# AIBluefisher/DReg-NeRF

Hardware: AMD Instinct MI355X
Metric: nerf_pairs_per_sec_regtr_fwd_bwd_128 (higher is better)
Workload: dtype bf16; 1 GPU; RegTR fwd+bwd+AdamW, shell-R synthetic pairs, 128^3 grids, 4 pairs (8 grids) per GPU per step, random-init weights; global_batch_pairs=4, resolution=128, fpn_head=active-set (identical results; rows around occupied voxels), parallelism=dp1

## Files before the change

### dreg_nerf_amd/csrc/pointset_exec.hip

```cpp
#include <hip/hip_runtime.h>
#include <cstdint>
#include <cstring>
#include <algorithm>
#include <vector>
#include "../../include/dreg_nerf.h"
#ifndef DREG_ELAUNCH
#define DREG_ELAUNCH (-2)
#endif

namespace {

constexpr int E = 256, E3 = 768, FF = 1024, NL = 6, NH = 8;
enum { N1W, N1B, SIW, SIB, SOW, SOB, N2W, N2B, CIW, CIB, COW, COB, N3W, N3B, L1W, L1B, L2W, L2B, PL_COUNT };
enum { FNW = NL * PL_COUNT, FNB, QW, QB, KW, KB, CW, CB, PS_NPARAM };
enum { LIN_SI, LIN_SO, LIN_CI, LIN_CO, LIN_1, LIN_2, LIN_PER_LAYER };
constexpr int NLIN = NL * LIN_PER_LAYER + 2;

struct Lin { int cout, cin, w, b; };
struct ReduceRec { const float* part; float* dw; int nsplit, Cout, Kpad, ntaps, Cin, Cin_real, accumulate, block0; };
static_assert(sizeof(ReduceRec) == 48, "matches WgradReduceDesc of conv.hip");
struct ColsumRec { const void* g; float* out; float* partial; int M, C, rpc, nch, pblock0, fblock0, accumulate, pad; };
static_assert(sizeof(ColsumRec) == 56, "matches ColsumDesc of fpn_ops.hip");
struct LnRec { const float* part; float* dg; float* db; int nblk, accumulate; };
static_assert(sizeof(LnRec) == 32, "matches LnFinalDesc of pointset.hip");

inline size_t al(size_t v) { return (v + 255) / 256 * 256; }

struct LayerBuf {
    size_t xa, xb, st1, st2, st3, h1, h2, h3, qkv1, qkv2, o1, o2, lse1, lse2, f;
    size_t gF, gB, gQ2, gC, gQ1;
    size_t wg[LIN_PER_LAYER], cs[LIN_PER_LAYER], lnp[3];
};
struct Layout {
    int R = -1;
    size_t allx, stf, dec_in, q, k, corr_lse;
    LayerBuf L[NL];
    size_t dallx, dallx_bf, dq, dk, ddec, ddec2, dH, dO, dvec, gx[2], lnpf[2], wgq, wgk, csq, csk, ov_ws, ks_ws, cs_ws, tables;
    size_t ks_bytes = 0, total = 0;
    size_t wg_bytes[NLIN];
};

struct Ps {
    float* val[PS_NPARAM];
    float* grad[PS_NPARAM];
    Lin lin[NLIN];
    Layout lay;
    int fuse = 1;
    int group_wgrad = 1;
    std::vector<hipEvent_t> ev;
    hipEvent_t ev_done = nullptr;
    static constexpr int RING = 8;
    static constexpr size_t TABLE_BYTES = 16384;
    char* pinned = nullptr;
    hipEvent_t ring_ev[RING] = {};
    unsigned ring_next = 0;
    struct Timed { hipEvent_t e0, e1; int kind, rows, cin, cout, flags; };
    bool timing = false;
    std::vector<Timed> timed;
    size_t timed_used = 0;
};

struct PsScope {
    Ps::Timed* t = nullptr; hipStream_t st;
    PsScope(Ps* p, void* stream, int kind, int rows, int cin, int cout, int flags) : st((hipStream_t)stream) {
        if (!p->timing) return;
        if (p->timed_used == p->timed.size()) {
            Ps::Timed n{};
            if (hipEventCreate(&n.e0) != hipSuccess || hipEventCreate(&n.e1) != hipSuccess) return;
            p->timed.push_back(n);
        }
        t = &p->timed[p->timed_used++];
        t->kind = kind; t->rows = rows; t->cin = cin; t->cout = cout; t->flags = flags;
        (void)hipEventRecord(t->e0, st);
    }
    ~PsScope() { if (t) (void)hipEventRecord(t->e1, st); }
};

inline int lin_index(int layer, int which) { return layer * LIN_PER_LAYER + which; }

void build_layout(Ps* p, int R)
{
    Layout& y = p->lay;
    if (y.R == R) return;
    y = Layout();
    y.R = R;
    size_t off = 0;
    auto take = [&](size_t bytes) { const size_t o = off; off += al(bytes); return o; };
    const size_t r = (size_t)R;
    y.allx = take(NL * r * E * 4);
    y.stf = take(NL * r * 2 * 4);
    y.dec_in = take(NL * r * E * 2);
    y.q = take(NL * r * E * 2);
    y.k = take(NL * r * E * 2);
    y.corr_lse = take(NL * r * 4);
    for (int i = 0; i < NLIN; ++i) {
        const Lin& l = p->lin[i];
        const int rows = i < NL * LIN_PER_LAYER ? R : NL * R;
        y.wg_bytes[i] = dreg_conv3d_wgrad_workspace_bytes(rows, 1, 1, 1, l.cin, l.cout, 1, 0);
        const size_t k1 = dreg_conv3d_igemm_workspace_bytes(rows, 1, 1, 1, l.cin, 1, 1, 1, l.cout, 1, 1, 0, 0, 0, 0);
        const size_t k2 = dreg_conv3d_igemm_workspace_bytes(rows, 1, 1, 1, l.cout, 1, 1, 1, l.cin, 1, 1, 0, 1, 0, 0);
// ... 39 lines not shown
int linear_fwd(Ps* p, const Layout& y, char* A, const void* x, const void* wpk, const float* bias, const void* residual, void* out,
               int rows, int cin, int cout, int relu, int out_f32, void* st)
{
    PsScope sc(p, st, 0, rows, cin, cout, (residual ? 1 : 0) | (out_f32 ? 2 : 0) | (y.ks_bytes ? 4 : 0));
    return dreg_conv3d_igemm_ws(x, wpk, out, bias, residual, rows, 1, 1, 1, cin, 1, 1, 1, cout, 1, 1, 0, 0, relu, residual ? 1 : 0, residual ? 1 : 0,
                                residual ? 1 : 0, residual ? 1 : 0, 0, out_f32, y.ks_bytes ? A + y.ks_ws : nullptr, y.ks_bytes, st);
}
int linear_dgrad(Ps* p, const Layout& y, char* A, const void* g, const void* wpk_t, void* gx, const void* mask, const void* add,
                 int rows, int cin, int cout, void* st)
{
    const void* addend = mask ? mask : add;
    PsScope sc(p, st, 1, rows, cin, cout, (addend ? 1 : 0) | (y.ks_bytes ? 4 : 0));
    return dreg_conv3d_igemm_ws(g, wpk_t, gx, nullptr, addend, rows, 1, 1, 1, cout, 1, 1, 1, cin, 1, 1, 0, 1, mask ? 2 : 0, addend ? 1 : 0, addend ? 1 : 0,
                                addend ? 1 : 0, addend ? 1 : 0, 0, 0, y.ks_bytes ? A + y.ks_ws : nullptr, y.ks_bytes, st);
}

}

extern "C" {

int dreg_ps_num_params(void) { return PS_NPARAM; }
int dreg_ps_num_linears(void) { return NLIN; }

void* dreg_ps_create(const int64_t* params)
{
    Ps* p = new Ps();
    for (int i = 0; i < PS_NPARAM; ++i) { p->val[i] = (float*)params[2 * i]; p->grad[i] = (float*)params[2 * i + 1]; }
    for (int l = 0; l < NL; ++l) {
        const int o = l * PL_COUNT;
        p->lin[lin_index(l, LIN_SI)] = {E3, E, o + SIW, o + SIB};
        p->lin[lin_index(l, LIN_SO)] = {E, E, o + SOW, o + SOB};
        p->lin[lin_index(l, LIN_CI)] = {E3, E, o + CIW, o + CIB};
        p->lin[lin_index(l, LIN_CO)] = {E, E, o + COW, o + COB};
        p->lin[lin_index(l, LIN_1)] = {FF, E, o + L1W, o + L1B};
        p->lin[lin_index(l, LIN_2)] = {E, FF, o + L2W, o + L2B};
    }
    p->lin[NLIN - 2] = {E, E, QW, QB};
    p->lin[NLIN - 1] = {E, E, KW, KB};
    if (hipHostMalloc((void**)&p->pinned, Ps::RING * Ps::TABLE_BYTES, hipHostMallocDefault) != hipSuccess) { delete p; return nullptr; }
    return p;
}
void dreg_ps_destroy(void* h)
{
    Ps* p = (Ps*)h;
    if (!p) return;
    for (auto& e : p->ev) if (e) (void)hipEventDestroy(e);
    if (p->ev_done) (void)hipEventDestroy(p->ev_done);
    for (auto& e : p->ring_ev) if (e) (void)hipEventDestroy(e);
    for (auto& t : p->timed) { (void)hipEventDestroy(t.e0); (void)hipEventDestroy(t.e1); }
    if (p->pinned) (void)hipHostFree(p->pinned);
    delete p;
}
void dreg_ps_set_fuse(void* h, int fuse) { ((Ps*)h)->fuse = fuse ? 1 : 0; }
void dreg_ps_set_group_wgrad(void* h, int on) { ((Ps*)h)->group_wgrad = on ? 1 : 0; }
void dreg_ps_set_timing(void* h, int enable) { ((Ps*)h)->timing = enable != 0; }
int dreg_ps_read_timings(void* h, int* info, float* ms, int cap)
{
    Ps* p = (Ps*)h;
    int n = 0;
    for (size_t i = 0; i < p->timed_used && n < cap; ++i) {
        const Ps::Timed& t = p->timed[i];
        float v = 0.f;
        if (hipEventElapsedTime(&v, t.e0, t.e1) != hipSuccess) continue;
        info[5 * n] = t.kind; info[5 * n + 1] = t.rows; info[5 * n + 2] = t.cin; info[5 * n + 3] = t.cout; info[5 * n + 4] = t.flags;
        ms[n++] = v;
    }
    p->timed_used = 0;
    return n;
}
size_t dreg_ps_arena_bytes(void* h, int R) { Ps* p = (Ps*)h; build_layout(p, R); return p->lay.total; }

int dreg_ps_forward(void* h, void* arena, size_t arena_bytes, const int64_t* packs, const float* feats, const float* xyz, const float* pe,
                    const int* probs_self, const int* probs_cross, int nprob, int max_len, int R,
                    float* cond, float* corr, float* ov, void* stream)
{
    Ps* p = (Ps*)h;
    if (R <= 0) return DREG_EINVAL;
    build_layout(p, R);
    const Layout& y = p->lay;
    if (arena_bytes < y.total) return DREG_EINVAL;
    char* A = (char*)arena;
    const float sc = 0.17677669529663687f;
    auto pk = [&](int li, int t) { return (const void*)packs[2 * li + t]; };
    const float* xin = feats;
    for (int l = 0; l < NL; ++l) {
        const LayerBuf& b = y.L[l];
        const int o = l * PL_COUNT;
        float* xout = (float*)(A + y.allx) + (size_t)l * R * E;
        CK(dreg_layernorm_fwd(xin, p->val[o + N1W], p->val[o + N1B], pe, A + b.h1, (float*)(A + b.st1), R, E, 1e-5f, 0, stream));
        CK(linear_fwd(p, y, A, A + b.h1, pk(lin_index(l, LIN_SI), 0), p->val[o + SIB], nullptr, A + b.qkv1, R, E, E3, 0, 0, stream));
        CK(dreg_mha_varlen_fwd(A + b.qkv1, A + b.qkv1 + E * 2, A + b.qkv1 + 2 * E * 2, A + b.o1, (float*)(A + b.lse1), probs_self, nprob, max_len, max_len,
                               R, NH, E3, E3, E3, E, sc, 0, stream));
        CK(linear_fwd(p, y, A, A + b.o1, pk(lin_index(l, LIN_SO), 0), p->val[o + SOB], xin, A + b.xa, R, E, E, 0, 1, stream));
        CK(dreg_layernorm_fwd((const float*)(A + b.xa), p->val[o + N2W], p->val[o + N2B], pe, A + b.h2, (float*)(A + b.st2), R, E, 1e-5f, 0, stream));
        CK(linear_fwd(p, y, A, A + b.h2, pk(lin_index(l, LIN_CI), 0), p->val[o + CIB], nullptr, A + b.qkv2, R, E, E3, 0, 0, stream));
        CK(dreg_mha_varlen_fwd(A + b.qkv2, A + b.qkv2 + E * 2, A + b.qkv2 + 2 * E * 2, A + b.o2, (float*)(A + b.lse2), probs_cross, nprob, max_len, max_len,
                               R, NH, E3, E3, E3, E, sc, 0, stream));
        CK(linear_fwd(p, y, A, A + b.o2, pk(lin_index(l, LIN_CO), 0), p->val[o + COB], A + b.xa, A + b.xb, R, E, E, 0, 1, stream));
        CK(dreg_layernorm_fwd((const float*)(A + b.xb), p->val[o + N3W], p->val[o + N3B], nullptr, A + b.h3, (float*)(A + b.st3), R, E, 1e-5f, 0, stream));
        CK(linear_fwd(p, y, A, A + b.h3, pk(lin_index(l, LIN_1), 0), p->val[o + L1B], nullptr, A + b.f, R, E, FF, 1, 0, stream));
        CK(linear_fwd(p, y, A, A + b.f, pk(lin_index(l, LIN_2), 0), p->val[o + L2B], A + b.xb, xout, R, FF, E, 0, 1, stream));
        xin = xout;
    }
    const int R6 = NL * R;
    CK(dreg_layernorm_fwd2((const float*)(A + y.allx), p->val[FNW], p->val[FNB], pe, R, cond, A + y.dec_in, (float*)(A + y.stf), R6, E, 1e-5f, stream));
    CK(linear_fwd(p, y, A, A + y.dec_in, pk(NLIN - 2, 0), p->val[QB], nullptr, A + y.q, R6, E, E, 0, 0, stream));
    CK(linear_fwd(p, y, A, A + y.dec_in, pk(NLIN - 1, 0), p->val[KB], nullptr, A + y.k, R6, E, E, 0, 0, stream));
    CK(dreg_corr_attention_varlen_fwd(A + y.q, A + y.k, xyz, corr, (float*)(A + y.corr_lse), probs_cross, nprob, max_len, max_len, NL, R, 0.0625f, 0, stream));
    CK(dreg_overlap_fwd(cond, p->val[CW], p->val[CB], ov, R6, stream));
    return DREG_OK;
}

int dreg_ps_backward(void* h, void* arena, size_t arena_bytes, const int64_t* packs, const float* feats, const float* xyz, const float* pe,
                     const int* probs_self, const int* probs_cross, int nprob, int max_len, int R,
                     const float* cond, const float* corr, const float* ov, const float* g_cond, const float* g_corr, const float* g_ov,
                     float* d_feats, void* stream, void* aux_stream, int last_only)
{
    Ps* p = (Ps*)h;
    if (R <= 0 || R != p->lay.R) return DREG_EINVAL;
    const Layout& y = p->lay;
    if (arena_bytes < y.total) return DREG_EINVAL;
    for (int i = 0; i < PS_NPARAM; ++i) if (!p->grad[i]) return DREG_EINVAL;
    char* A = (char*)arena;
    hipStream_t st = (hipStream_t)stream;
    hipStream_t ax = aux_stream && aux_stream != stream ? (hipStream_t)aux_stream : st;
    const bool two = ax != st;
    const float sc = 0.17677669529663687f;
    const int LB = last_only ? NL - 1 : 0, nlb = last_only ? 1 : NL;
    const int R6 = nlb * R;
    const size_t rb = (size_t)LB * R;
    const int fuse = p->fuse;
    auto pk = [&](int li, int t) { return (const void*)packs[2 * li + t]; };
    cond += rb * E; corr += rb * 3; ov += rb;
    if (p->ev.size() < (size_t)NLIN + 2) {
        p->ev.resize(NLIN + 2, nullptr);
        for (auto& e : p->ev) if (!e && hipEventCreateWithFlags(&e, hipEventDisableTiming) != hipSuccess) return DREG_ELAUNCH;
        if (hipEventCreateWithFlags(&p->ev_done, hipEventDisableTiming) != hipSuccess) return DREG_ELAUNCH;
    }
    std::vector<ReduceRec> rd;
    std::vector<ColsumRec> cs;
    std::vector<LnRec> ln;
    int rd_blocks = 0, cs_p = 0, cs_f = 0;
    struct GroupRec { char d[160]; int variant, nblocks; };
    std::vector<GroupRec> grp;
    const bool group = fuse && p->group_wgrad && !p->timing;
    auto param_grads = [&](int li, const void* g, const void* x, int rows, size_t wg_off, size_t cs_off) -> int {
        const Lin& l = p->lin[li];
        bool grouped = false;
        if (group) {
            GroupRec gr{};
            if (dreg_linear_wgrad_group_fill(gr.d, g, x, A + wg_off, y.wg_bytes[li], rows, l.cin, l.cout, &gr.variant, &gr.nblocks) == DREG_OK) { grp.push_back(gr); grouped = true; }
        }
        if (!grouped) {
            if (two) { if (hipEventRecord(p->ev[li], st) != hipSuccess || hipStreamWaitEvent(ax, p->ev[li], 0) != hipSuccess) return DREG_ELAUNCH; }
// ... 153 lines not shown
```

### dreg_nerf_amd/lib.py

```python
import ctypes
import os
from ctypes import c_float, c_int, c_size_t, c_void_p

import torch

_HERE = os.path.dirname(os.path.abspath(__file__))
LIB_PATH = os.path.join(_HERE, "libdreg_nerf_hip.so")

DT_BF16 = 0
DT_F32 = 1

_lib = None


class DregError(RuntimeError):
    pass


def _sig(lib, name, restype, argtypes):
    fn = getattr(lib, name)
    fn.restype = restype
    fn.argtypes = argtypes
    return fn

# ... 94 lines not shown
    "dreg_pack_rgba_grids_occ": (I, [P, P, P, I, I, I, I, I, P]),
    "dreg_pack_rgba_sparse": (I, [P, P, P, P, I, I, I, I, I, I, P]),
    "dreg_pack_rgba_sparse_occ": (I, [P, P, P, P, P, I, I, I, I, I, I, P]),
    "dreg_conv_row_occupancy": (I, [P, P, I, I, I, I, I, I, I, I, P]),
    "dreg_gather_grid_xyz": (I, [P, P, P, P, I, I, I, I, P]),
    "dreg_exec_create": (P, [P, I, P, I, P, I]),
    "dreg_exec_destroy": (None, [P]),
    "dreg_exec_op_halo": (I, [P, I]),
    "dreg_exec_arena_bytes": (Z, [P]),
    "dreg_exec_pack_bytes": (Z, [P]),
    "dreg_exec_num_packs": (I, [P]),
    "dreg_exec_tensor_offset": (Z, [P, I]),
    "dreg_exec_output_slot": (I, [P]),
    "dreg_exec_pack_rows": (I, [P]),
    "dreg_exec_export_pack_table": (I, [P, P, P, P]),
    "dreg_exec_repack": (I, [P, P, P, P]),
    "dreg_exec_set_overlap": (None, [P, I]),
    "dreg_exec_set_input_row_occupancy": (None, [P, P]),
    "dreg_exec_set_timing": (None, [P, I]),
    "dreg_exec_read_timings": (I, [P, P, P, I]),
    "dreg_exec_forward": (I, [P, P, Z, P, P, P, I, I, P]),
    "dreg_exec_backward": (I, [P, P, Z, P, P, P, P, I, P, P]),
    "dreg_exec_backward_range": (I, [P, P, Z, P, P, P, P, I, P, P, I, I, I]),
    "dreg_mha_fwd": (I, [P] * 5 + [I] * 7 + [F, I, P]),
    "dreg_mha_bwd": (I, [P] * 10 + [I] * 7 + [F, I, P]),
    "dreg_corr_attention_fwd": (I, [P] * 5 + [I] * 3 + [F, I, P]),
    "dreg_corr_attention_bwd": (I, [P] * 9 + [I] * 3 + [F, I, P]),
    "dreg_mha_varlen_fwd": (I, [P] * 6 + [I] * 9 + [F, I, P]),
    "dreg_mha_varlen_bwd": (I, [P] * 11 + [I] * 9 + [F, I, P]),
    "dreg_corr_attention_varlen_fwd": (I, [P] * 6 + [I] * 5 + [F, I, P]),
    "dreg_corr_attention_varlen_bwd": (I, [P] * 10 + [I] * 5 + [F, I, P]),
    "dreg_layernorm_fwd": (I, [P] * 6 + [I, I, F, I, P]),
    "dreg_layernorm_bwd_workspace_bytes": (Z, [I]),
    "dreg_layernorm_bwd": (I, [P] * 8 + [I] * 5 + [P]),
    "dreg_layernorm_bwd_add": (I, [P] * 9 + [I] * 4 + [P]),
    "dreg_layernorm_fwd2": (I, [P, P, P, P, I, P, P, P, I, I, F, P]),
    "dreg_layernorm_bwd_parts": (I, [P] * 10 + [I, I, I, P]),
    "dreg_layernorm_bwd_blocks": (I, [I]),
    "dreg_layernorm_bwd_final_batched": (I, [P, I, P]),
    "dreg_overlap_bwd_acc": (I, [P, P, P, P, P, P, P, P, I, P, I, P]),
    "dreg_colsum_rows_per_chunk": (I, [Z]),
    "dreg_colsum_batched": (I, [P, I, I, I, P]),
    "dreg_brick_supported": (I, [I] * 6),
    "dreg_conv3_brick_pack_bytes": (Z, [I, I]),
    "dreg_pack_conv_weight_brick": (I, [P, P, I, I, I, P]),
    "dreg_brick_tiles_workspace_bytes": (Z, [I] * 4),
    "dreg_brick_tiles_build": (I, [P, I, I, I, I, I, I, P, Z, P, P, P, P, P, P]),
    "dreg_conv3_brick": (I, [P, P, P, P, P, P, I, P, P, P] + [I] * 11 + [P]),
    "dreg_ps_num_params": (I, []),
    "dreg_ps_num_linears": (I, []),
    "dreg_ps_create": (P, [P]),
    "dreg_ps_destroy": (None, [P]),
    "dreg_ps_set_fuse": (None, [P, I]),
    "dreg_ps_set_timing": (None, [P, I]),
    "dreg_ps_read_timings": (I, [P, P, P, I]),
    "dreg_ps_arena_bytes": (Z, [P, I]),
    "dreg_ps_forward": (I, [P, P, Z, P, P, P, P, P, P, I, I, I, P, P, P, P]),
    "dreg_ps_backward": (I, [P, P, Z, P, P, P, P, P, P, I, I, I, P, P, P, P, P, P, P, P, P, I]),
    "dreg_posenc_sine": (I, [P, P, I, F, F, P]),
    "dreg_overlap_fwd": (I, [P, P, P, P, I, P]),
    "dreg_overlap_bwd_workspace_bytes": (Z, [I]),
    "dreg_overlap_bwd": (I, [P] * 8 + [I, P]),
    "dreg_relu_bwd": (I, [P, P, P, Z, I, I, I, P]),
    "dreg_weighted_kabsch": (I, [P, P, P, P, I, I, F, P]),
    "dreg_weighted_kabsch_pairs": (I, [P, P, P, P, P, I, I, I, F, P]),
    "dreg_weighted_kabsch_bwd": (I, [P] * 7 + [I, I, F, P]),
    "dreg_weighted_kabsch_pairs_bwd": (I, [P] * 7 + [I, I, I, F, P]),
    "dreg_reg_point_losses": (I, [P] * 10 + [I, I, I, I, F, F, F, P]),
    "dreg_infonce_nn": (I, [P] * 7 + [I, I, F, P]),
    "dreg_infonce_rows": (I, [P] * 10 + [I, I, F, F, I, P]),
    "dreg_reg_losses_final": (I, [P] * 6 + [I, I, F, F, F, F, F, P]),
    "dreg_nerf_cont_deferred": (I, [P] * 5 + [I, I, I, F, F, F, F, P]),
    "dreg_halfspace_labels": (I, [P, P, P, P, I, I, P]),
    "dreg_voxel_downsample_workspace_bytes": (Z, [I]),
    "dreg_voxel_downsample_fwd": (I, [P] * 11 + [Z, I, I, I, F, P]),
    "dreg_voxel_downsample_bwd": (I, [P, P, P, P, I, I, P]),
    "dreg_voxel_downsample_plan": (I, [P] * 11 + [Z, I, I, F, P]),
    "dreg_voxel_downsample_plan_frozen": (I, [P] * 11 + [Z, I, I, F, P, P]),
    "dreg_voxel_segment_mean": (I, [P] * 5 + [I, I, P]),
    "dreg_grad_norm": (I, [P, P, P, Z, P]),
    "dreg_adamw_step": (I, [P] * 5 + [Z] + [F] * 5 + [I, F, P]),
    "dreg_ngp_level_table": (ctypes.c_uint32, [F, I, I, P, P, P, P, P]),
    "dreg_f32_to_f16": (I, [P, P, Z, P]),
    "dreg_ngp_density_fwd": (I, [P] * 6 + [P] * 5 + [P, I, P]),
    "dreg_ngp_rgb_mean_fwd": (I, [P] * 6 + [I, I, P]),
    "dreg_ngp_dir_bias": (I, [P, P, P, I, P]),
    "dreg_ngp_alpha_keep": (I, [P, P, P, I, F, F, P]),
    "dreg_ngp_density_fwd_contract": (I, [P] * 6 + [P] * 5 + [P, I, I, P]),
    "dreg_ngp_density_fwd_ws": (I, [P] * 6 + [P] * 5 + [P, I, I, P, Z, P, I, P]),
    "dreg_grid_sample_points_ordered": (I, [P, P, P, P, P, I, I, I, P, I, P]),
    "dreg_grid_x_order_workspace_bytes": (Z, [I, I, I]),
    "dreg_grid_x_order": (I, [P, P, P, P, Z, I, I, I, I, P]),
    "dreg_grid_occupied_workspace_bytes": (Z, [I, I, I]),
    "dreg_grid_occupied_totals": (P, [P, I, I, I]),
    "dreg_grid_occupied_count": (I, [P, P, Z, I, I, I, P]),
    "dreg_grid_occupied_build": (I, [P, P, P, P, P, P, P, P, I, I, I, I, P]),
    "dreg_ngp_density_keep_fwd_ws": (I, [P] * 6 + [P] * 5 + [P, I, I, P, Z, P, I] + [P, P, F, F, P]),
    "dreg_grid_write_kept": (I, [P, P, P, P, P, P, P, P, I, I, I, I, P]),
    "dreg_ngp_density_workspace_bytes": (Z, [I]),
    "dreg_ngp_rgb_dir_fwd": (I, [P] * 6 + [I, P]),
    "dreg_grid_scatter7": (I, [P] * 6 + [I, P]),
    "dreg_grid_sample_points": (I, [P, P, P, I, I, I, P, I, P]),
    "dreg_surface_visibility": (I, [P] * 7 + [P] * 5 + [P, P, P] + [I] * 5 + [F, F, F, F, P]),
    "dreg_surface_visibility_queue": (I, [P] * 7 + [P] * 5 + [P, P, P] + [I] * 5 + [F, F, F, F, P, P, P]),
    "dreg_occupancy_coarse_bits": (I, [P, P, I, I, I, P]),
    "dreg_surface_visibility_desc_bytes": (Z, []),
# ... 169 lines not shown
```

### dreg_nerf_amd/pointset_exec.py

```python
import ctypes
from typing import Dict, Optional

import numpy as np
import torch

from . import lib as L
from . import ops

N_LAYERS = 6
_PER_LAYER = ("norm1.weight", "norm1.bias", "self_attn.in_proj_weight", "self_attn.in_proj_bias", "self_attn.out_proj.weight",
              "self_attn.out_proj.bias", "norm2.weight", "norm2.bias", "cross_attn.in_proj_weight", "cross_attn.in_proj_bias",
              "cross_attn.out_proj.weight", "cross_attn.out_proj.bias", "norm3.weight", "norm3.bias", "linear1.weight", "linear1.bias",
              "linear2.weight", "linear2.bias")
_TAIL = ("transformer_encoder.norm.weight", "transformer_encoder.norm.bias", "correspondence_decoder.q_proj.weight",
         "correspondence_decoder.q_proj.bias", "correspondence_decoder.k_proj.weight", "correspondence_decoder.k_proj.bias",
         "correspondence_decoder.conf_logits_decoder.weight", "correspondence_decoder.conf_logits_decoder.bias")
_LINEARS = ("self_attn.in_proj_weight", "self_attn.out_proj.weight", "cross_attn.in_proj_weight", "cross_attn.out_proj.weight",
            "linear1.weight", "linear2.weight")

FUSE = True
GROUP_WGRAD = True


def param_names():
    names = [f"transformer_encoder.layers.{l}.{n}" for l in range(N_LAYERS) for n in _PER_LAYER]
    return names + list(_TAIL)


def linear_names():
    names = [f"transformer_encoder.layers.{l}.{n}" for l in range(N_LAYERS) for n in _LINEARS]
    return names + ["correspondence_decoder.q_proj.weight", "correspondence_decoder.k_proj.weight"]


class PointSetExecutor:

    def __init__(self, P: Dict[str, torch.Tensor], with_grad: bool):
        self.lib = L.load()
        names = param_names()
        assert len(names) == self.lib.dreg_ps_num_params()
        self.params = [P[n] for n in names]
        self.linears = [P[n] for n in linear_names()]
        assert len(self.linears) == self.lib.dreg_ps_num_linears()
        self.with_grad = with_grad
        tab = np.zeros((len(names), 2), dtype=np.int64)
        self._sig = []
        for i, t in enumerate(self.params):
            assert t.is_contiguous() and t.dtype == torch.float32, "the executor reads fp32 master parameters in place"
            g = t.grad if with_grad else None
            if with_grad and (g is None or not g.is_contiguous() or g.dtype != torch.float32):
                raise L.DregError("PointSetExecutor needs preallocated contiguous fp32 .grad buffers (FlatAdamW) on every parameter")
            tab[i, 0] = t.data_ptr()
            tab[i, 1] = g.data_ptr() if g is not None else 0
            self._sig.append((t.data_ptr(), int(tab[i, 1])))
        self.h = self.lib.dreg_ps_create(tab.ctypes.data)
        if not self.h:
            raise L.DregError("dreg_ps_create failed")
        self.lib.dreg_ps_set_fuse(self.h, int(FUSE))
        self.lib.dreg_ps_set_group_wgrad(self.h, int(GROUP_WGRAD))
        self._fuse = FUSE
        self._group = GROUP_WGRAD
        self.device = self.params[0].device
        self.arena = None
        self.arena_bytes = 0
        self._timing = False
        self._packs = (ctypes.c_int64 * (2 * len(self.linears)))()
        self._pack_stamp = None
        self._pack_keep = None

    def __del__(self):
        try:
            if getattr(self, "h", None):
                self.lib.dreg_ps_destroy(self.h)
                self.h = None
        except Exception:
            pass

    def still_valid(self) -> bool:
        for t, (vp, gp) in zip(self.params, self._sig):
            g = t.grad if self.with_grad else None
            if t.data_ptr() != vp or (g.data_ptr() if g is not None else 0) != gp:
                return False
        return True

    def _pack_table(self):
        stamp = (ops._weight_generation, sum(t._version for t in self.linears))
        if stamp != self._pack_stamp:
            keep = []
            for i, w in enumerate(self.linears):
                f = ops.packed_weight(w, w.shape[1], False, L.DT_BF16)
                d = ops.packed_weight(w, w.shape[1], True, L.DT_BF16)
                self._packs[2 * i], self._packs[2 * i + 1] = f.data_ptr(), d.data_ptr()
                keep += [f, d]
            self._pack_keep, self._pack_stamp = keep, stamp
        return ctypes.addressof(self._packs)

    def _arena_for(self, R: int):
        need = self.lib.dreg_ps_arena_bytes(self.h, R)
        if need > self.arena_bytes:
            self.arena = None
            self.arena_bytes = int(need * 1.25)
            self.arena = torch.empty(self.arena_bytes, dtype=torch.uint8, device=self.device)
        return self.arena

    def set_timing(self, on: bool):
        self._timing = bool(on)
        self.lib.dreg_ps_set_timing(self.h, int(on))

    def drain_timings(self, profiler: "ops.KernelTimer"):
        cap = 4096
        info = (ctypes.c_int * (5 * cap))()
        ms = (ctypes.c_float * cap)()
        n = self.lib.dreg_ps_read_timings(self.h, info, ms, cap)
        for i in range(n):
            kind, rows, cin, cout, flags = (info[5 * i + k] for k in range(5))
            fl = 2.0 * rows * cin * cout
            if kind == 2:
                var = self.lib.dreg_conv3d_wgrad_variant(rows, 1, 1, 1, cin, cout, 1, 0, 0, 0)
                name = "conv_wgrad_glds_kernel<256,256,false,8>" if var == 256256 else f"conv_wgrad_glds_kernel<{var // 1000},{var % 1000},false,4>"
                label = f"wgrad B{rows} 1x1x1x{cin} g1x1x1x{cout} k1s1"
            elif kind == 1:
                name = ops.igemm_kernel_name(self.lib, rows, 1, 1, 1, cout, 1, 1, 1, cin, 1, 1, 0, 1, 0, bool(flags & 4), bool(flags & 1), L.DT_BF16, False)
                label = f"dgrad B{rows} 1x1x1x{cout}->1x1x1x{cin} k1s1"
            else:
                name = ops.igemm_kernel_name(self.lib, rows, 1, 1, 1, cin, 1, 1, 1, cout, 1, 1, 0, 0, 0, bool(flags & 4), bool(flags & 1), L.DT_BF16, bool(flags & 2))
                label = f"fwd B{rows} 1x1x1x{cin}->1x1x1x{cout} k1s1"
            profiler.add_measured(name, label, fl, ms[i])

    def forward(self, feats, xyz, pe, tab):
        if self._fuse != FUSE:
            self.lib.dreg_ps_set_fuse(self.h, int(FUSE))
            self._fuse = FUSE
        if self._group != GROUP_WGRAD:
            self.lib.dreg_ps_set_group_wgrad(self.h, int(GROUP_WGRAD))
            self._group = GROUP_WGRAD
        want = ops.PROFILER is not None and ops.PROFILER.enabled
        if want != self._timing:
            self.set_timing(want)
        ops.wait_packs()
        R = feats.shape[0]
        arena = self._arena_for(R)
        dev = feats.device
        cond = torch.empty(N_LAYERS, R, 256, dtype=torch.float32, device=dev)
        corr = torch.empty(N_LAYERS, R, 3, dtype=torch.float32, device=dev)
        ov = torch.empty(N_LAYERS, R, 1, dtype=torch.float32, device=dev)
        L.check(self.lib.dreg_ps_forward(self.h, L.ptr(arena), self.arena_bytes, self._pack_table(), L.ptr(feats), L.ptr(xyz), L.ptr(pe),
                                         L.ptr(tab.self_probs), L.ptr(tab.cross_probs), tab.nprob, tab.max_len, R,
                                         L.ptr(cond), L.ptr(corr), L.ptr(ov), L.stream()), "dreg_ps_forward")
        self.generation = getattr(self, "generation", 0) + 1
        return cond, corr, ov

    def backward(self, feats, xyz, pe, tab, cond, corr, ov, g_cond, g_corr, g_ov, last_only=False, generation=None):
        if generation is not None and generation != getattr(self, "generation", 0):
            raise L.DregError("PointSetExecutor.backward: the shared arena was overwritten by a later forward pass (two grad-mode forwards before a "
                              "backward: gradient accumulation over several forwards / retain_graph need one executor per live graph)")
        R = feats.shape[0]
        d_feats = torch.empty_like(feats)
        aux = None if self._timing else ops.PARAM_GRAD_STREAM
        if aux is not None:
            self.arena.record_stream(aux)
        L.check(self.lib.dreg_ps_backward(self.h, L.ptr(self.arena), self.arena_bytes, self._pack_table(), L.ptr(feats), L.ptr(xyz), L.ptr(pe),
                                          L.ptr(tab.self_probs), L.ptr(tab.cross_probs), tab.nprob, tab.max_len, R,
                                          L.ptr(cond), L.ptr(corr), L.ptr(ov), L.ptr(g_cond), L.ptr(g_corr), L.ptr(g_ov), L.ptr(d_feats),
                                          L.stream(), aux.cuda_stream if aux is not None else None, int(last_only)), "dreg_ps_backward")
        return d_feats


class _PointSetFn(torch.autograd.Function):

    @staticmethod
    def forward(ctx, feats, anchor, ex: PointSetExecutor, xyz, pe, tab):
        cond, corr, ov = ex.forward(feats, xyz, pe, tab)
        ctx.ex, ctx.tab, ctx.generation = ex, tab, ex.generation
        ctx.save_for_backward(feats, xyz, pe, cond, corr, ov)
        ctx.set_materialize_grads(False)
        return cond, corr, ov, cond[-1].clone(), corr[-1].clone(), ov[-1].clone()

    @staticmethod
    def backward(ctx, g_cond, g_corr, g_ov, g_cl, g_rl, g_ol):
        feats, xyz, pe, cond, corr, ov = ctx.saved_tensors
        f32 = lambda g: g.contiguous().float() if g is not None else None
        if FUSE and g_cond is None and g_corr is None and g_ov is None:
            d_feats = ctx.ex.backward(feats, xyz, pe, ctx.tab, cond, corr, ov, f32(g_cl), f32(g_rl), f32(g_ol), last_only=True, generation=ctx.generation)
            return d_feats, None, None, None, None, None
        full = []
        for g, gl, ref in ((g_cond, g_cl, cond), (g_corr, g_rl, corr), (g_ov, g_ol, ov)):
            if gl is not None:
                g = torch.zeros_like(ref) if g is None else g.contiguous().float().clone()
# ... 30 lines not shown
```

### include/dreg_nerf.h

```cpp
#ifndef DREG_NERF_H
#define DREG_NERF_H
#include <stddef.h>
#include <stdint.h>

#ifdef __cplusplus
extern "C" {
#endif

#define DREG_OK 0
#define DREG_EINVAL (-1)

int dreg_conv_get_glds(void);


int dreg_conv3d_kpad(int ksz, int Cin, int dtype);

int dreg_pack_conv_weight(const float* w, void* out, int Cout, int Cin_real, int Cin, int ksz, int for_dgrad,
                          int dtype, void* stream);
int dreg_pack_conv_weights_batched(const void* descs, int n, int total_rows, int stage_floats, const int* row_desc,
                                   void* stream);

int dreg_conv3d_igemm(const void* in, const void* wt_packed, void* out, const float* bias, const void* addend,
                      int B, int Di, int Hi, int Wi, int Cin, int Do, int Ho, int Wo, int Cout,
                      int ksz, int stride, int pad, int transposed, int relu, int Da, int Ha, int Wa, int add_same,
// ... 368 lines not shown
                                  const void* table, const void* w1, const void* w2,
                                  const uint32_t* offset, const uint32_t* size, const uint32_t* res, const float* scale, const uint32_t* hashed,
                                  const float* roi_aabb, const float* scene_aabb, const float* model_aabb,
                                  int rx, int ry, int rz, int Nc, int Np, float render_step_size, float cut_off, float early_stop_eps,
                                  float alpha_thre, void* queue, const uint32_t* coarse_bits, void* stream);
int dreg_occupancy_coarse_bits(const uint8_t* binary, uint32_t* bits, int rx, int ry, int rz, void* stream);
size_t dreg_surface_visibility_desc_bytes(void);
int dreg_surface_visibility_fill_desc(void* host_desc, const float* cams, const float* pts, const uint8_t* binary, int* label,
                                      const void* table, const void* w1, const void* w2,
                                      const uint32_t* offset, const uint32_t* size, const uint32_t* res, const float* scale, const uint32_t* hashed,
                                      const float* roi_aabb, const float* scene_aabb, const float* model_aabb,
                                      int rx, int ry, int rz, int Nc, int Np, float render_step_size, float cut_off, float early_stop_eps,
                                      float alpha_thre, void* queue, const uint32_t* coarse_bits);
int dreg_surface_visibility_multi(const void* descs_dev, int n, long total_rays, void* stream);
int dreg_surface_visibility_multi_waves(const void* descs_dev, int n, long total_rays, int max_waves, void* stream);

int dreg_ngp_render(const float* origins, const float* viewdirs, long n_rays, const uint8_t* binary, int rx, int ry, int rz, const uint32_t* coarse_bits,
                    const void* table, const void* w1, const void* w2, const void* cw1, const void* cw2, const void* cw3,
                    const uint32_t* offset, const uint32_t* size, const uint32_t* res, const float* scale, const uint32_t* hashed,
                    const float* roi_aabb, const float* scene_aabb, const float* model_aabb, float near_plane, float far_plane,
                    float render_step_size, float alpha_thre, float early_stop_eps, const float* bkgd,
                    float* rgb, float* opacity, float* depth, unsigned long long* n_samples, void* queue, void* stream);

int dreg_ngp_render_train(const float* origins, const float* viewdirs, const float* jitter, long n_rays, const uint8_t* binary, int rx, int ry, int rz,
                          const uint32_t* coarse_bits, const void* table, const void* w1, const void* w2, const void* cw1, const void* cw2, const void* cw3,
                          const uint32_t* offset, const uint32_t* size, const uint32_t* res, const float* scale, const uint32_t* hashed,
                          const float* roi_aabb, const float* scene_aabb, const float* model_aabb, float near_plane, float far_plane,
                          float render_step_size, float alpha_thre, float early_stop_eps, const float* bkgd,
                          float* rgb, float* opacity, float* depth, unsigned long long* n_samples, void* queue, void* stream);
size_t dreg_ngp_render_bwd_workspace_bytes(long n_rays);
int dreg_ngp_render_bwd(const float* origins, const float* viewdirs, const float* jitter, long n_rays, const uint8_t* binary, int rx, int ry, int rz,
                        const uint32_t* coarse_bits, const void* base16, const void* color16,
                        const uint32_t* offset, const uint32_t* size, const uint32_t* res, const float* scale, const uint32_t* hashed,
                        const float* roi_aabb, const float* scene_aabb, const float* model_aabb, float near_plane, float far_plane,
                        float render_step_size, float alpha_thre, float early_stop_eps,
                        const float* rgb, const float* grad_rgb, float* grad_base, float* grad_color, void* workspace, size_t workspace_bytes, void* stream);
int dreg_ngp_adam_step(float* p, float* g, float* m, float* v, void* p16, size_t n, float lr, float beta1, float beta2, float eps, int step, void* stream);

int dreg_brick_supported(int B, int D, int H, int W, int Cin, int Cout);
size_t dreg_conv3_brick_pack_bytes(int rows, int red);
int dreg_pack_conv_weight_brick(const float* w, void* out, int Cout, int Cin, int transposed, void* stream);
size_t dreg_brick_tiles_workspace_bytes(int B, int D, int H, int W);
int dreg_brick_tiles_build(const uint8_t* flags, int B, int D, int H, int W, int max_rows, int max_tiles, void* workspace, size_t workspace_bytes,
                           int* meta, int* rows_sorted, void* tiles, int* halo_vox, void* nbr, void* stream);
int dreg_conv3_brick(const void* in, const void* wpk, void* out, const float* bias, const void* addend, const void* tiles, int ntiles,
                     const int* halo_vox, const void* nbr, const int* rows_sorted,
                     int B, int D, int H, int W, int Cin, int Cout, int Da, int Ha, int Wa, int add_same, int out_f32, void* stream);

int dreg_ps_num_params(void);
int dreg_ps_num_linears(void);
void* dreg_ps_create(const int64_t* params);
void dreg_ps_destroy(void* h);
void dreg_ps_set_fuse(void* h, int fuse);
void dreg_ps_set_group_wgrad(void* h, int on);
void dreg_ps_set_timing(void* h, int enable);
int dreg_ps_read_timings(void* h, int* info, float* ms, int cap);
size_t dreg_ps_arena_bytes(void* h, int R);
int dreg_ps_forward(void* h, void* arena, size_t arena_bytes, const int64_t* packs, const float* feats, const float* xyz, const float* pe,
                    const int* probs_self, const int* probs_cross, int nprob, int max_len, int R,
                    float* cond, float* corr, float* ov, void* stream);
int dreg_ps_backward(void* h, void* arena, size_t arena_bytes, const int64_t* packs, const float* feats, const float* xyz, const float* pe,
                     const int* probs_self, const int* probs_cross, int nprob, int max_len, int R,
                     const float* cond, const float* corr, const float* ov, const float* g_cond, const float* g_corr, const float* g_ov,
                     float* d_feats, void* stream, void* aux_stream, int last_only);

#ifdef __cplusplus
}
#endif
#endif
```

Baseline: 256.2 pairs/s.

## Fuse point-set transformer forward chains into two row-block megakernels

Adds two fused forward kernels for the point-set transformer layers. Chain A fuses the self-attention out-projection, residual add, LayerNorm and cross-attention QKV projection. Chain B fuses the cross out-projection, residual, LayerNorm, both FFN linears and the next layer's LayerNorm plus QKV projection, keeping each 64-row block in LDS. This cuts kernel launches and global round-trips of intermediates in the forward pass. In exchange, rows now pass through a single block with large LDS use, which may lower occupancy relative to the tuned standalone GEMMs.

```diff
diff --git a/dreg_nerf_amd/csrc/pointset_chain.h b/dreg_nerf_amd/csrc/pointset_chain.h
--- /dev/null
+++ b/dreg_nerf_amd/csrc/pointset_chain.h
@@ -0,0 +1,22 @@
+#pragma once
+#include <hip/hip_runtime.h>
+#include "common.h"
+
+namespace dreg_chain {
+
+struct Args {
+    const bf16_t* attn;
+    const bf16_t* w_out; const float* b_out;
+    const float* res; float* x;
+    const float* ln_g; const float* ln_b; const float* ln_pe; bf16_t* h; float* st;
+    const bf16_t* w_qkv; const float* b_qkv; bf16_t* qkv;
+    const bf16_t* w1; const float* b1; bf16_t* f;
+    const bf16_t* w2; const float* b2; float* x2;
+    const float* ln1_g; const float* ln1_b; const float* ln1_pe; bf16_t* h1; float* st1;
+    int R;
+};
+
+__attribute__((visibility("hidden"))) int launch_a(const Args& a, hipStream_t st);
+__attribute__((visibility("hidden"))) int launch_b(const Args& a, hipStream_t st);
+
+}
diff --git a/dreg_nerf_amd/csrc/pointset_chain.hip b/dreg_nerf_amd/csrc/pointset_chain.hip
--- /dev/null
+++ b/dreg_nerf_amd/csrc/pointset_chain.hip
@@ -0,0 +1,237 @@
+#include "pointset_chain.h"
+#include "../../include/dreg_nerf.h"
+
+namespace dreg_chain {
+namespace {
+
+constexpr int BM = 64, NW = 8, NT = NW * 64, E = 256, E3 = 768, FF = 1024;
+constexpr int A_BYTES = BM * E * 2;
+constexpr int C_BYTES = BM * E * 4;
+
+__device__ __forceinline__ uint32_t a_off(int row, int gran) { return (uint32_t)row * 512u + (uint32_t)((gran ^ (row & 15)) << 4); }
+__device__ __forceinline__ uint32_t c_off(int row, int gran) { return (uint32_t)row * 1024u + (uint32_t)((gran ^ (row & 15)) << 4); }
+
+struct Half { bf16x8_t v[4][2]; };
+typedef f32x4_t Acc[4][2];
+
+__device__ __forceinline__ void load_half(Half& f, const bf16_t* w, int ldk, int wave, int lane)
+{
+    const int fr = lane & 15, kg = lane >> 4;
+    const bf16_t* p = w + (size_t)(wave * 32 + fr) * ldk + kg * 8;
+#pragma unroll
+    for (int j = 0; j < 2; ++j)
+#pragma unroll
+        for (int ks = 0; ks < 4; ++ks) f.v[ks][j] = *reinterpret_cast<const bf16x8_t*>(p + (size_t)j * 16 * ldk + ks * 32);
+}
+__device__ __forceinline__ void mma_half(Acc& acc, const char* sA, int gran0, const Half& f, int lane)
+{
+    const int fr = lane & 15, kg = lane >> 4;
+#pragma unroll
+    for (int ks = 0; ks < 4; ++ks) {
+        bf16x8_t af[4];
+#pragma unroll
+        for (int i = 0; i < 4; ++i) af[i] = *reinterpret_cast<const bf16x8_t*>(sA + a_off(i * 16 + fr, gran0 + ks * 4 + kg));
+#pragma unroll
+        for (int i = 0; i < 4; ++i)
+#pragma unroll
+            for (int j = 0; j < 2; ++j) acc[i][j] = __builtin_amdgcn_mfma_f32_16x16x32_bf16(f.v[ks][j], af[i], acc[i][j], 0, 0, 0);
+    }
+}
+template <bool NEXT>
+__device__ __forceinline__ void gemm256(Acc& acc, const char* sA, const bf16_t* w, int ldk, const bf16_t* w_next, int ldk_next, Half& f0, int wave, int lane)
+{
+    Half f1;
+    load_half(f1, w + 128, ldk, wave, lane);
+    __builtin_amdgcn_sched_barrier(0);
+    mma_half(acc, sA, 0, f0, lane);
+    __builtin_amdgcn_sched_barrier(0);
+    if constexpr (NEXT) load_half(f0, w_next, ldk_next, wave, lane);
+    __builtin_amdgcn_sched_barrier(0);
+    mma_half(acc, sA, 16, f1, lane);
+    __builtin_amdgcn_sched_barrier(0);
+}
+__device__ __forceinline__ void zero(Acc& acc)
+{
+#pragma unroll
+    for (int i = 0; i < 4; ++i)
+#pragma unroll
+        for (int j = 0; j < 2; ++j) acc[i][j] = (f32x4_t){0.f, 0.f, 0.f, 0.f};
+}
+__device__ __forceinline__ void acc_to_lds(const Acc& acc, char* sC, int wave, int lane)
+{
+    const int rl = lane & 15, gq = lane >> 4;
+#pragma unroll
+    for (int i = 0; i < 4; ++i)
+#pragma unroll
+        for (int j = 0; j < 2; ++j) *reinterpret_cast<f32x4_t*>(sC + c_off(i * 16 + rl, wave * 8 + j * 4 + gq)) = acc[i][j];
+}
+__device__ __forceinline__ void load_block(char* sA, const bf16_t* src, int m0, int R, int t)
+{
+    uint4 v[BM / 16];
+    const int gran = t & 31;
+#pragma unroll
+    for (int p = 0; p < BM / 16; ++p) {
+        const int r = p * 16 + (t >> 5);
+        v[p] = make_uint4(0u, 0u, 0u, 0u);
+        if (m0 + r < R) v[p] = *reinterpret_cast<const uint4*>(src + (size_t)(m0 + r) * E + gran * 8);
+    }
+    __builtin_amdgcn_sched_barrier(0);
+#pragma unroll
+    for (int p = 0; p < BM / 16; ++p) *reinterpret_cast<uint4*>(sA + a_off(p * 16 + (t >> 5), gran)) = v[p];
+}
+
+__device__ __forceinline__ void rows_res_ln(const char* sC, char* sA, const float* bias, const float* res, float* x, bool ln, const float* g,
+                                            const float* b, const float* pe, bf16_t* h, float* st, int m0, int R, int wave, int lane)
+{
+    const float4 bi = *reinterpret_cast<const float4*>(bias + lane * 4);
+    float4 gg = make_float4(0.f, 0.f, 0.f, 0.f), bb = gg;
+    if (ln) { gg = *reinterpret_cast<const float4*>(g + lane * 4); bb = *reinterpret_cast<const float4*>(b + lane * 4); }
+    float4 rv[8], pv[8];
+#pragma unroll
+    for (int u = 0; u < 8; ++u) {
+        const int row = m0 + wave * 8 + u;
+        rv[u] = make_float4(0.f, 0.f, 0.f, 0.f); pv[u] = rv[u];
+        if (row < R) {
+            rv[u] = *reinterpret_cast<const float4*>(res + (size_t)row * E + lane * 4);
+            if (ln && pe) pv[u] = *reinterpret_cast<const float4*>(pe + (size_t)row * E + lane * 4);
+        }
+    }
+#pragma unroll
+    for (int u = 0; u < 8; ++u) {
+        const int lr = wave * 8 + u, row = m0 + lr;
+        if (row >= R) continue;
+        const float4 c = *reinterpret_cast<const float4*>(sC + c_off(lr, lane));
+        float4 v;
+        v.x = c.x + bi.x; v.y = c.y + bi.y; v.z = c.z + bi.z; v.w = c.w + bi.w;
+        v.x += rv[u].x; v.y += rv[u].y; v.z += rv[u].z; v.w += rv[u].w;
+        *reinterpret_cast<float4*>(x + (size_t)row * E + lane * 4) = v;
+        if (!ln) continue;
+        const float mean = wave_sum(v.x + v.y + v.z + v.w) * (1.f / 256.f);
+        const float d0 = v.x - mean, d1 = v.y - mean, d2 = v.z - mean, d3 = v.w - mean;
+        const float var = wave_sum(d0 * d0 + d1 * d1 + d2 * d2 + d3 * d3) * (1.f / 256.f);
+        const float rstd = 1.0f / sqrtf(var + 1e-5f);
+        float o[4] = {d0 * rstd * gg.x + bb.x, d1 * rstd * gg.y + bb.y, d2 * rstd * gg.z + bb.z, d3 * rstd * gg.w + bb.w};
+        if (pe) { o[0] += pv[u].x; o[1] += pv[u].y; o[2] += pv[u].z; o[3] += pv[u].w; }
+        const uint2 q = make_uint2(f2bf2(o[0], o[1]), f2bf2(o[2], o[3]));
+        *reinterpret_cast<uint2*>(h + (size_t)row * E + lane * 4) = q;
+        *reinterpret_cast<uint2*>(sA + a_off(lr, lane >> 1) + (lane & 1) * 8) = q;
+        if (lane == 0) { st[2 * row] = mean; st[2 * row + 1] = rstd; }
+    }
+}
+template <bool RELU>
+__device__ __forceinline__ void rows_bf16(const char* sC, char* sA, const float* bias, bf16_t* out, int ldo, int m0, int R, int wave, int lane)
+{
+    const float4 bi = *reinterpret_cast<const float4*>(bias + lane * 4);
+#pragma unroll
+    for (int u = 0; u < 8; ++u) {
+        const int lr = wave * 8 + u, row = m0 + lr;
+        if (row >= R) continue;
+        const float4 c = *reinterpret_cast<const float4*>(sC + c_off(lr, lane));
+        float v[4] = {c.x + bi.x, c.y + bi.y, c.z + bi.z, c.w + bi.w};
+        if constexpr (RELU) {
+#pragma unroll
+            for (int e = 0; e < 4; ++e) v[e] = fmaxf(v[e], 0.f);
+        }
+        const uint2 q = make_uint2(f2bf2(v[0], v[1]), f2bf2(v[2], v[3]));
+        *reinterpret_cast<uint2*>(out + (size_t)row * ldo + lane * 4) = q;
+        if (sA) *reinterpret_cast<uint2*>(sA + a_off(lr, lane >> 1) + (lane & 1) * 8) = q;
+    }
+}
+
+__device__ __forceinline__ void front(const Args& a, char* sA, char* sC, Half& f0, const bf16_t* w_next, int ldk_next, int m0, int wave, int lane)
+{
+    Acc acc;
+    zero(acc);
+    gemm256<true>(acc, sA, a.w_out, E, w_next, ldk_next, f0, wave, lane);
+    acc_to_lds(acc, sC, wave, lane);
+    __syncthreads();
+    rows_res_ln(sC, sA, a.b_out, a.res, a.x, true, a.ln_g, a.ln_b, a.ln_pe, a.h, a.st, m0, a.R, wave, lane);
+    __syncthreads();
+}
+__device__ __forceinline__ void in_proj(const Args& a, const char* sA, char* sC, Half& f0, int m0, int wave, int lane)
+{
+#pragma unroll
+    for (int nc = 0; nc < 3; ++nc) {
+        Acc acc;
+        zero(acc);
+        const bf16_t* w = a.w_qkv + (size_t)nc * 256 * E;
+        if (nc < 2) gemm256<true>(acc, sA, w, E, w + (size_t)256 * E, E, f0, wave, lane);
+        else gemm256<false>(acc, sA, w, E, nullptr, 0, f0, wave, lane);
+        acc_to_lds(acc, sC, wave, lane);
+        __syncthreads();
+        rows_bf16<false>(sC, nullptr, a.b_qkv + nc * 256, a.qkv + nc * 256, E3, m0, a.R, wave, lane);
+        if (nc < 2) __syncthreads();
+    }
+}
+
+}
+
+__global__ __launch_bounds__(NT) void ps_chain_a_kernel(Args a)
+{
+    extern __shared__ __attribute__((aligned(16))) char smem[];
+    char* sA = smem;
+    char* sC = smem + A_BYTES;
+    const int t = threadIdx.x, lane = t & 63, wave = __builtin_amdgcn_readfirstlane(t >> 6);
+    const int m0 = blockIdx.x * BM;
+    Half f0;
+    load_half(f0, a.w_out, E, wave, lane);
+    load_block(sA, a.attn, m0, a.R, t);
+    __syncthreads();
+    front(a, sA, sC, f0, a.w_qkv, E, m0, wave, lane);
+    in_proj(a, sA, sC, f0, m0, wave, lane);
+}
+
+__global__ __launch_bounds__(NT) void ps_chain_b_kernel(Args a)
+{
+    extern __shared__ __attribute__((aligned(16))) char smem[];
+    char* sA = smem;
+    char* sF = smem + A_BYTES;
+    char* sC = smem + 2 * A_BYTES;
+    const int t = threadIdx.x, lane = t & 63, wave = __builtin_amdgcn_readfirstlane(t >> 6);
+    const int m0 = blockIdx.x * BM;
+    const bool has_next = a.w_qkv != nullptr;
+    Half f0;
+    load_half(f0, a.w_out, E, wave, lane);
+    load_block(sA, a.attn, m0, a.R, t);
+    __syncthreads();
+    front(a, sA, sC, f0, a.w1, E, m0, wave, lane);
+    Acc acc2;
+    zero(acc2);
+#pragma unroll 1
+    for (int c = 0; c < 4; ++c) {
+        Acc acc1;
+        zero(acc1);
+        gemm256<true>(acc1, sA, a.w1 + (size_t)c * 256 * E, E, a.w2 + c * 256, FF, f0, wave, lane);
+        acc_to_lds(acc1, sC, wave, lane);
+        __syncthreads();
+        rows_bf16<true>(sC, sF, a.b1 + c * 256, a.f + c * 256, FF, m0, a.R, wave, lane);
+        __syncthreads();
+        const bf16_t* wn = c < 3 ? a.w1 + (size_t)(c + 1) * 256 * E : (has_next ? a.w_qkv : a.w_out);
+        gemm256<true>(acc2, sF, a.w2 + c * 256, FF, wn, E, f0, wave, lane);
+    }
+    acc_to_lds(acc2, sC, wave, lane);
+    __syncthreads();
+    rows_res_ln(sC, sA, a.b2, a.x, a.x2, has_next, a.ln1_g, a.ln1_b, a.ln1_pe, a.h1, a.st1, m0, a.R, wave, lane);
+    if (!has_next) return;
+    __syncthreads();
+    in_proj(a, sA, sC, f0, m0, wave, lane);
+}
+
+int launch_a(const Args& a, hipStream_t st)
+{
+    constexpr int lds = A_BYTES + C_BYTES;
+    (void)hipFuncSetAttribute((const void*)ps_chain_a_kernel, hipFuncAttributeMaxDynamicSharedMemorySize, lds);
+    hipLaunchKernelGGL(ps_chain_a_kernel, dim3((a.R + BM - 1) / BM), dim3(NT), (size_t)lds, st, a);
+    DREG_LAUNCH_CHECK();
+    return DREG_OK;
+}
+int launch_b(const Args& a, hipStream_t st)
+{
+    constexpr int lds = 2 * A_BYTES + C_BYTES;
+    (void)hipFuncSetAttribute((const void*)ps_chain_b_kernel, hipFuncAttributeMaxDynamicSharedMemorySize, lds);
+    hipLaunchKernelGGL(ps_chain_b_kernel, dim3((a.R + BM - 1) / BM), dim3(NT), (size_t)lds, st, a);
+    DREG_LAUNCH_CHECK();
+    return DREG_OK;
+}
+
+}
diff --git a/dreg_nerf_amd/csrc/pointset_exec.hip b/dreg_nerf_amd/csrc/pointset_exec.hip
--- a/dreg_nerf_amd/csrc/pointset_exec.hip
+++ b/dreg_nerf_amd/csrc/pointset_exec.hip
@@ -4,6 +4,7 @@
 #include <algorithm>
 #include <vector>
 #include "../../include/dreg_nerf.h"
+#include "pointset_chain.h"
 #ifndef DREG_ELAUNCH
 #define DREG_ELAUNCH (-2)
 #endif
@@ -46,6 +47,7 @@
     Lin lin[NLIN];
     Layout lay;
     int fuse = 1;
+    int chain = 3;
     int group_wgrad = 1;
     std::vector<hipEvent_t> ev;
     hipEvent_t ev_done = nullptr;
@@ -191,6 +193,7 @@
     delete p;
 }
 void dreg_ps_set_fuse(void* h, int fuse) { ((Ps*)h)->fuse = fuse ? 1 : 0; }
+void dreg_ps_chain_mask(void* h, int mask) { ((Ps*)h)->chain = mask & 3; }
 void dreg_ps_set_group_wgrad(void* h, int on) { ((Ps*)h)->group_wgrad = on ? 1 : 0; }
 void dreg_ps_set_timing(void* h, int enable) { ((Ps*)h)->timing = enable != 0; }
 int dreg_ps_read_timings(void* h, int* info, float* ms, int cap)
@@ -222,23 +225,56 @@
     const float sc = 0.17677669529663687f;
     auto pk = [&](int li, int t) { return (const void*)packs[2 * li + t]; };
     const float* xin = feats;
+    const int chain = p->fuse ? p->chain : 0;
     for (int l = 0; l < NL; ++l) {
         const LayerBuf& b = y.L[l];
         const int o = l * PL_COUNT;
         float* xout = (float*)(A + y.allx) + (size_t)l * R * E;
-        CK(dreg_layernorm_fwd(xin, p->val[o + N1W], p->val[o + N1B], pe, A + b.h1, (float*)(A + b.st1), R, E, 1e-5f, 0, stream));
-        CK(linear_fwd(p, y, A, A + b.h1, pk(lin_index(l, LIN_SI), 0), p->val[o + SIB], nullptr, A + b.qkv1, R, E, E3, 0, 0, stream));
+        if (l == 0 || !(chain & 2)) {
+            CK(dreg_layernorm_fwd(xin, p->val[o + N1W], p->val[o + N1B], pe, A + b.h1, (float*)(A + b.st1), R, E, 1e-5f, 0, stream));
+            CK(linear_fwd(p, y, A, A + b.h1, pk(lin_index(l, LIN_SI), 0), p->val[o + SIB], nullptr, A + b.qkv1, R, E, E3, 0, 0, stream));
+        }
         CK(dreg_mha_varlen_fwd(A + b.qkv1, A + b.qkv1 + E * 2, A + b.qkv1 + 2 * E * 2, A + b.o1, (float*)(A + b.lse1), probs_self, nprob, max_len, max_len,
                                R, NH, E3, E3, E3, E, sc, 0, stream));
-        CK(linear_fwd(p, y, A, A + b.o1, pk(lin_index(l, LIN_SO), 0), p->val[o + SOB], xin, A + b.xa, R, E, E, 0, 1, stream));
-        CK(dreg_layernorm_fwd((const float*)(A + b.xa), p->val[o + N2W], p->val[o + N2B], pe, A + b.h2, (float*)(A + b.st2), R, E, 1e-5f, 0, stream));
-        CK(linear_fwd(p, y, A, A + b.h2, pk(lin_index(l, LIN_CI), 0), p->val[o + CIB], nullptr, A + b.qkv2, R, E, E3, 0, 0, stream));
+        if (chain & 1) {
+            dreg_chain::Args a{};
+            a.attn = (const bf16_t*)(A + b.o1); a.w_out = (const bf16_t*)pk(lin_index(l, LIN_SO), 0); a.b_out = p->val[o + SOB];
+            a.res = xin; a.x = (float*)(A + b.xa);
+            a.ln_g = p->val[o + N2W]; a.ln_b = p->val[o + N2B]; a.ln_pe = pe; a.h = (bf16_t*)(A + b.h2); a.st = (float*)(A + b.st2);
+            a.w_qkv = (const bf16_t*)pk(lin_index(l, LIN_CI), 0); a.b_qkv = p->val[o + CIB]; a.qkv = (bf16_t*)(A + b.qkv2);
+            a.R = R;
+            PsScope scope(p, stream, 3, R, E, E + E3, 0);
+            CK(dreg_chain::launch_a(a, (hipStream_t)stream));
+        } else {
+            CK(linear_fwd(p, y, A, A + b.o1, pk(lin_index(l, LIN_SO), 0), p->val[o + SOB], xin, A + b.xa, R, E, E, 0, 1, stream));
+            CK(dreg_layernorm_fwd((const float*)(A + b.xa), p->val[o + N2W], p->val[o + N2B], pe, A + b.h2, (float*)(A + b.st2), R, E, 1e-5f, 0, stream));
+            CK(linear_fwd(p, y, A, A + b.h2, pk(lin_index(l, LIN_CI), 0), p->val[o + CIB], nullptr, A + b.qkv2, R, E, E3, 0, 0, stream));
+        }
         CK(dreg_mha_varlen_fwd(A + b.qkv2, A + b.qkv2 + E * 2, A + b.qkv2 + 2 * E * 2, A + b.o2, (float*)(A + b.lse2), probs_cross, nprob, max_len, max_len,
                                R, NH, E3, E3, E3, E, sc, 0, stream));
-        CK(linear_fwd(p, y, A, A + b.o2, pk(lin_index(l, LIN_CO), 0), p->val[o + COB], A + b.xa, A + b.xb, R, E, E, 0, 1, stream));
-        CK(dreg_layernorm_fwd((const float*)(A + b.xb), p->val[o + N3W], p->val[o + N3B], nullptr, A + b.h3, (float*)(A + b.st3), R, E, 1e-5f, 0, stream));
-        CK(linear_fwd(p, y, A, A + b.h3, pk(lin_index(l, LIN_1), 0), p->val[o + L1B], nullptr, A + b.f, R, E, FF, 1, 0, stream));
-        CK(linear_fwd(p, y, A, A + b.f, pk(lin_index(l, LIN_2), 0), p->val[o + L2B], A + b.xb, xout, R, FF, E, 0, 1, stream));
+        if (chain & 2) {
+            const bool next = l + 1 < NL;
+            dreg_chain::Args a{};
+            a.attn = (const bf16_t*)(A + b.o2); a.w_out = (const bf16_t*)pk(lin_index(l, LIN_CO), 0); a.b_out = p->val[o + COB];
+            a.res = (const float*)(A + b.xa); a.x = (float*)(A + b.xb);
+            a.ln_g = p->val[o + N3W]; a.ln_b = p->val[o + N3B]; a.ln_pe = nullptr; a.h = (bf16_t*)(A + b.h3); a.st = (float*)(A + b.st3);
+            a.w1 = (const bf16_t*)pk(lin_index(l, LIN_1), 0); a.b1 = p->val[o + L1B]; a.f = (bf16_t*)(A + b.f);
+            a.w2 = (const bf16_t*)pk(lin_index(l, LIN_2), 0); a.b2 = p->val[o + L2B]; a.x2 = xout;
+            if (next) {
+                const LayerBuf& n = y.L[l + 1];
+                const int on = (l + 1) * PL_COUNT;
+                a.ln1_g = p->val[on + N1W]; a.ln1_b = p->val[on + N1B]; a.ln1_pe = pe; a.h1 = (bf16_t*)(A + n.h1); a.st1 = (float*)(A + n.st1);
+                a.w_qkv = (const bf16_t*)pk(lin_index(l + 1, LIN_SI), 0); a.b_qkv = p->val[on + SIB]; a.qkv = (bf16_t*)(A + n.qkv1);
+            }
+            a.R = R;
+            PsScope scope(p, stream, 4, R, E, E + 2 * FF + (next ? E3 : 0), 0);
+            CK(dreg_chain::launch_b(a, (hipStream_t)stream));
+        } else {
+            CK(linear_fwd(p, y, A, A + b.o2, pk(lin_index(l, LIN_CO), 0), p->val[o + COB], A + b.xa, A + b.xb, R, E, E, 0, 1, stream));
+            CK(dreg_layernorm_fwd((const float*)(A + b.xb), p->val[o + N3W], p->val[o + N3B], nullptr, A + b.h3, (float*)(A + b.st3), R, E, 1e-5f, 0, stream));
+            CK(linear_fwd(p, y, A, A + b.h3, pk(lin_index(l, LIN_1), 0), p->val[o + L1B], nullptr, A + b.f, R, E, FF, 1, 0, stream));
+            CK(linear_fwd(p, y, A, A + b.f, pk(lin_index(l, LIN_2), 0), p->val[o + L2B], A + b.xb, xout, R, FF, E, 0, 1, stream));
+        }
         xin = xout;
     }
     const int R6 = NL * R;
diff --git a/dreg_nerf_amd/lib.py b/dreg_nerf_amd/lib.py
--- a/dreg_nerf_amd/lib.py
+++ b/dreg_nerf_amd/lib.py
@@ -170,6 +170,7 @@
     "dreg_ps_create": (P, [P]),
     "dreg_ps_destroy": (None, [P]),
     "dreg_ps_set_fuse": (None, [P, I]),
+    "dreg_ps_chain_mask": (None, [P, I]),
     "dreg_ps_set_timing": (None, [P, I]),
     "dreg_ps_read_timings": (I, [P, P, P, I]),
     "dreg_ps_arena_bytes": (Z, [P, I]),
diff --git a/dreg_nerf_amd/pointset_exec.py b/dreg_nerf_amd/pointset_exec.py
--- a/dreg_nerf_amd/pointset_exec.py
+++ b/dreg_nerf_amd/pointset_exec.py
@@ -19,6 +19,7 @@
             "linear1.weight", "linear2.weight")
 
 FUSE = True
+CHAIN = 3
 GROUP_WGRAD = True
 
 
@@ -57,8 +58,10 @@
             raise L.DregError("dreg_ps_create failed")
         self.lib.dreg_ps_set_fuse(self.h, int(FUSE))
         self.lib.dreg_ps_set_group_wgrad(self.h, int(GROUP_WGRAD))
+        self.lib.dreg_ps_chain_mask(self.h, int(CHAIN))
         self._fuse = FUSE
         self._group = GROUP_WGRAD
+        self._chain = CHAIN
         self.device = self.params[0].device
         self.arena = None
         self.arena_bytes = 0
@@ -114,6 +117,10 @@
         for i in range(n):
             kind, rows, cin, cout, flags = (info[5 * i + k] for k in range(5))
             fl = 2.0 * rows * cin * cout
+            if kind in (3, 4):
+                name = "ps_chain_a_kernel" if kind == 3 else "ps_chain_b_kernel"
+                profiler.add_measured(name, f"fwd chain {'A' if kind == 3 else 'B'} B{rows} {cin}x{cout}", fl, ms[i])
+                continue
             if kind == 2:
                 var = self.lib.dreg_conv3d_wgrad_variant(rows, 1, 1, 1, cin, cout, 1, 0, 0, 0)
                 name = "conv_wgrad_glds_kernel<256,256,false,8>" if var == 256256 else f"conv_wgrad_glds_kernel<{var // 1000},{var % 1000},false,4>"
@@ -133,6 +140,9 @@
         if self._group != GROUP_WGRAD:
             self.lib.dreg_ps_set_group_wgrad(self.h, int(GROUP_WGRAD))
             self._group = GROUP_WGRAD
+        if self._chain != CHAIN:
+            self.lib.dreg_ps_chain_mask(self.h, int(CHAIN))
+            self._chain = CHAIN
         want = ops.PROFILER is not None and ops.PROFILER.enabled
         if want != self._timing:
             self.set_timing(want)
diff --git a/include/dreg_nerf.h b/include/dreg_nerf.h
--- a/include/dreg_nerf.h
+++ b/include/dreg_nerf.h
@@ -444,6 +444,7 @@
 void* dreg_ps_create(const int64_t* params);
 void dreg_ps_destroy(void* h);
 void dreg_ps_set_fuse(void* h, int fuse);
+void dreg_ps_chain_mask(void* h, int mask);
 void dreg_ps_set_group_wgrad(void* h, int on);
 void dreg_ps_set_timing(void* h, int enable);
 int dreg_ps_read_timings(void* h, int* info, float* ms, int cap);
```

Result: no change. 257.6 pairs/s (median of 6 runs) (+0.6%).
